# dropbox/rust-brotli

Measured on AMD Instinct MI355X. Metric: compress MB/s at q5 lgwin22, higher is better.
Workload: dtype u8; 1 GPU; 64 MiB synthetic English-like text per GPU, quality=5, lgwin=22, one-shot BrotliEncoderCompress (H6), input and stream resident in HBM; input_bytes_total=67108864, compressed_bytes=16370400

## Files before the change

### rust-brotli_amd/csrc/device_api.h

```cpp
#ifndef BROTLI_MI355X_DEVICE_API_H_
#define BROTLI_MI355X_DEVICE_API_H_

#include <stddef.h>
#include <stdint.h>

#include <vector>

#include "lz77_types.h"
#include "lz77_warmup.h"

#define BR_STREAM (::brotli_mi355x::dev_stream_flushed())

struct ihipStream_t;
namespace brotli_mi355x {

ihipStream_t* dev_stream_flushed();

void* dev_alloc(size_t bytes);
void* dev_alloc_uninit(size_t bytes);
#ifdef BROTLI_HOST_EMU
void dev_free(void* p);
#else
void dev_free(void* p) noexcept;
static_assert(noexcept(dev_free(nullptr)), "blocks are freed in destructors");
// ... 129 lines not shown
  uint16_t* stag;
  uint32_t* rows;
  void* checkpoints = nullptr;
  uint32_t* rows_changed_lo = nullptr;
  uint32_t* rows_changed_hi = nullptr;
  uint32_t splice_lists = 1;
  uint32_t* dict_items = nullptr;
  uint32_t* changed_slot;
  uint32_t* row_ctl;
  uint32_t* reset_counts;
  const uint32_t* count_base;
  uint32_t* run_end;
  unsigned long long* smask;
  uint32_t* gprev;
  uint8_t* big_tile;
  unsigned long long* pot = nullptr;
  uint32_t* pot_state = nullptr;
  uint32_t* pot_list = nullptr;
  uint32_t pot_list_cap = 0;
  uint32_t* flip_cells = nullptr;
  uint32_t cell_shift = 0, cells_per_key = 0;
  uint32_t changed_cap;
  uint16_t* sorted_tag[2] = {nullptr, nullptr};
  uint32_t* search_log = nullptr;
  uint32_t* recheck_list = nullptr;
  uint32_t* recheck_count = nullptr;
  uint32_t recheck_cap = 0;
  uint8_t* flags[2];
  Command* cmds;
  Segment* segments;
// ... 159 lines not shown
```

### rust-brotli_amd/csrc/lz77_kernels.hip

```cpp
#include <hip/hip_runtime.h>
#include <stdexcept>
#include <string>
#include <utility>
#include <string.h>
#include <mutex>
#include <vector>

#include "device_api.h"
#include "lz77_chain.h"
#include "lz77_rows.h"
#include "lz77_groups.h"
#include "device_scan.h"
#include "lz77_parse_args.h"
#include "zopfli_device.h"
#include "batch_greedy_device.h"

namespace brotli_mi355x {

void hip_check(hipError_t e, const char* what) {
  if (e == hipSuccess) return;
  (void)hipGetLastError();
  throw std::runtime_error(std::string("HIP error in ") + what + ": " + hipGetErrorString(e));
}

static constexpr uint32_t kSortTile = 4096;
// ... 654 lines not shown

__device__ __forceinline__ void row_changed(const RowArgs& a, uint32_t p) {
  if (p < a.geo.first_block_start) return;
  if (a.flags[p] & kFlagSearched) {
    mark_dirty(p, a.geo, a.dirty, a.rows_lo, a.rows_hi);
  } else {
    const uint32_t k = chain_in_front_if_near_boundary(p, a.geo);
    if (k != 0xffffffffu) {
      a.dirty[k] = 1;
      note_rows_changed(k, p, a.rows_lo, a.rows_hi);
    }
  }
}

static constexpr uint32_t kRowTile = kScanTile, kRowHalo = 256, kRowSpan = kRowTile + kRowHalo;
static constexpr uint32_t kMaxRowWalk = 2048;
static_assert(kRowSpan == 256 * 5, "five span entries per thread");

__global__ __launch_bounds__(256) void k_build_rows(RowArgs a) {
  if (a.conditional && a.ctl[kCtlNeedFull] == 0) return;
  if (a.conditional && a.validate && a.pot != nullptr && a.pot_state[0] != 0 && a.pot_state[2] == 0) return;
  typedef uint32_t u32x4 __attribute__((ext_vector_type(4)));
  __shared__ uint32_t s_pos[kRowSpan];
  __shared__ uint32_t s_tk[kRowSpan];
  __shared__ uint8_t s_fb[kRowSpan];
  __shared__ uint16_t s_rank[kRowSpan];
  __shared__ uint2 c_ent[kRowSpan];
  __shared__ uint32_t wave_sum[4];
  __shared__ alignas(16) uint32_t rowbuf[4][64 * kRowEntries];
  const uint32_t base = blockIdx.x * kRowTile;
// ... 223 lines not shown
        want = count != 0 && (count & 0xffffu) == 0;
      }
      if (want != ((f[j] & kSlotWrap) != 0)) {
        fbits[i] = (uint8_t)(f[j] ^ kSlotWrap);
        if (append) {
          const uint32_t real = *changed_count;
          const uint32_t at = real + atomicAdd(&ctl[kCtlVirtual], 1u);
          if (real <= cap && at < cap) changed_slot[at] = i; else atomicMax(&ctl[kCtlNeedFull], 1u);
        }
      }
    }
    g += f[j] & kSlotStored;
  }
}

__device__ __forceinline__ uint32_t slot_bits_of_flag(uint32_t flag) { return (flag & 1u) | ((flag & kFlagMasked) ? kSlotMasked : 0u); }

__global__ __launch_bounds__(256) void k_regather_fbits(const uint32_t* __restrict__ by_key, const uint8_t* __restrict__ flags, uint32_t n,
                                                         uint8_t* __restrict__ fbits, const uint32_t* __restrict__ ctl) {
  if (ctl[kCtlNeedFull] != 2) return;
  for (uint32_t i = blockIdx.x * blockDim.x + threadIdx.x; i < n; i += gridDim.x * blockDim.x)
    fbits[i] = (uint8_t)(slot_bits_of_flag(flags[by_key[i]]) | (fbits[i] & kSlotWrap));
}

__global__ __launch_bounds__(256) void k_apply_flips(const uint32_t* __restrict__ changed_pos, const uint32_t* __restrict__ changed_count,
                                                      uint32_t cap, const uint16_t* __restrict__ keys, const uint32_t* __restrict__ key_first,
                                                      const uint32_t* __restrict__ key_last, const uint32_t* __restrict__ by_key,
                                                      const uint8_t* __restrict__ flags_new, uint8_t* __restrict__ fbits,
                                                      uint32_t* __restrict__ changed_slot, uint32_t* __restrict__ ctl, uint32_t total_slots,
                                                      uint32_t all_keys) {
  const uint32_t i = blockIdx.x * blockDim.x + threadIdx.x;
  const uint32_t n = *changed_count;
  if (n > cap) {
    if (i == 0) {
      atomicMax(&ctl[kCtlNeedFull], 2u);
      atomicMax(&ctl[kCtlWrapKeyFlip], 1u);
    }
    return;
// ... 38 lines not shown
      const bool st = in && i != s && (a.fbits[i] & (kSlotStored | kSlotChanged)) == kSlotStored;
      const unsigned long long m = __ballot(st);
      const uint32_t before = (uint32_t)__popcll(m & ((1ull << threadIdx.x) - 1ull));
      bool build = in && stable + before < a.depth;
      if (use_pot && build) build = ((a.pot[i >> 6] >> (i & 63u)) & 1ull) != 0;
      if (build) {
        if (br_build_row(sl, a.rows, a.max_backward_limit, i, kf, a.depth, true, a.reset_pos, a.reset_vis)) row_changed(a, a.by_key[i]);
      }
      stable += (uint32_t)__popcll(m);
      const uint32_t cost = use_pot ? (__ballot(build) != 0 ? 64u : 4u) : 64u;
      if (threadIdx.x == 0) atomicAdd(&a.walk_counter[kCtlWalked], cost);
    }
  }
}

__global__ __launch_bounds__(256) void k_clear_flip_marks(const uint32_t* __restrict__ changed_slot, const uint32_t* __restrict__ changed_count,
                                                           uint32_t cap, uint8_t* __restrict__ fbits) {
  const uint32_t n = *changed_count;
  if (n > cap) return;
  for (uint32_t i = blockIdx.x * blockDim.x + threadIdx.x; i < n; i += gridDim.x * blockDim.x) fbits[changed_slot[i]] &= (uint8_t)~kSlotChanged;
}

static RowArgs row_args(const Lz77Params& P, const Lz77Buffers& B, int which, bool validate, const SegGeometry* geo, uint8_t* dirty_dev) {
  RowArgs a{};
  a.by_key = B.by_key;
  a.sorted_keys = B.sorted_keys;
  a.stag = B.stag;
  a.fbits = B.fbits;
  a.key_first = B.key_first;
  a.key_last = B.key_last;
  a.rows = B.rows;
  a.flags = B.flags[which];
  a.n = P.total_bytes;
  a.depth = 1u << P.block_bits;
  a.max_backward_limit = P.max_backward_limit;
// ... 14 lines not shown
  a.flip_cells = (validate && B.count_base == nullptr && P.reset_pos == 0) ? B.flip_cells : nullptr;
  a.cell_shift = B.cell_shift;
  a.cells_per_key = B.cells_per_key;
  a.cell_words = (uint32_t)(((size_t)65536 * B.cells_per_key) / 32);
  return a;
}

#if !defined(BR_POT_TABLE)
#define BR_POT_TABLE 8192
#define BR_POT_SHIFT 19
#endif
static constexpr uint32_t kPotTile = 1024, kPotHalo = 512, kPotSpan = kPotTile + kPotHalo, kPotTable = BR_POT_TABLE, kPotShift = BR_POT_SHIFT;
__global__ __launch_bounds__(256) void k_row_potential(const uint32_t* __restrict__ by_key, const uint16_t* __restrict__ sorted_keys,
                                                        const uint16_t* __restrict__ stag, uint32_t n, uint32_t max_backward_limit,
                                                        const uint32_t* __restrict__ ctl, uint32_t* __restrict__ pot_state,
                                                        unsigned long long* __restrict__ pot, uint32_t* __restrict__ pot_list, uint32_t list_cap) {
  if (ctl[kCtlNeedFull] == 0 || pot_state[0] != 0) return;
  __shared__ uint32_t s_val[kPotSpan];
  __shared__ uint32_t s_pos[kPotSpan];
  __shared__ uint32_t tab[kPotTable], tab2[kPotTable];
  __shared__ uint32_t s_count, s_base;
  const uint32_t lane = threadIdx.x & 63u;
  for (uint32_t h = threadIdx.x; h < kPotTable; h += 256) tab[h] = tab2[h] = 0;
  uint32_t gen = 0;
  for (uint32_t base = blockIdx.x * kPotTile; base < n; base += gridDim.x * kPotTile) {
    ++gen;
    const uint32_t lo = base >= kPotHalo ? base - kPotHalo : 0u;
    const uint32_t hi = min(base + kPotTile, n);
    const uint32_t span = hi - lo;
    __syncthreads();
    for (uint32_t e = threadIdx.x; e < span; e += 256) {
// ... 77 lines not shown
      }
      s_base = at;
    }
    __syncthreads();
    if (s_base != 0xffffffffu) {
      uint32_t at = s_base + (uint32_t)__shfl((int)wave_at, 0, 64);
#pragma unroll
      for (uint32_t r = 0; r < kPotTile / 256; ++r) {
        const unsigned long long m = masks[r];
        if ((m >> lane) & 1ull) pot_list[at + (uint32_t)__popcll(m & ((1ull << lane) - 1ull))] = base + r * 256 + threadIdx.x;
        at += (uint32_t)__popcll(m);
      }
    }
  }
}
__global__ __launch_bounds__(256) void k_validate_listed_rows(RowArgs a, const uint32_t* __restrict__ pot_list) {
  if (a.ctl[kCtlNeedFull] == 0 || a.pot_state[0] == 0 || a.pot_state[2] != 0) return;
  const uint32_t count = a.pot_state[1];
  SlotsInMemory sl{a.by_key, a.fbits, a.stag, a.smask, a.gprev};
  for (uint32_t t = blockIdx.x * blockDim.x + threadIdx.x; t < count; t += gridDim.x * blockDim.x) {
    const uint32_t i = pot_list[t];
    if (a.flip_cells != nullptr && a.flip_cells[a.cell_words] == 0) {
      const uint32_t p = a.by_key[i];
      const uint32_t first = (p > a.max_backward_limit ? p - a.max_backward_limit : 0u) >> a.cell_shift, last = p >> a.cell_shift;
      const uint32_t key = a.sorted_keys[i];
      const uint32_t cell0 = key * a.cells_per_key;
      bool any = a.key_last[key] - a.key_first[key] >= 65536u;
      for (uint32_t c = cell0 + first; c <= cell0 + last; ++c) any = any || ((a.flip_cells[c >> 5] >> (c & 31u)) & 1u) != 0;
      if (!any) continue;
    }
    const uint32_t kf = a.key_first[a.sorted_keys[i]];
    if (br_build_row(sl, a.rows, a.max_backward_limit, i, kf, a.depth, true, a.reset_pos, a.reset_vis)) row_changed(a, a.by_key[i]);
  }
}
__global__ void k_row_potential_ready(const uint32_t* __restrict__ ctl, uint32_t* __restrict__ pot_state) {
  if (ctl[kCtlNeedFull] != 0 && threadIdx.x == 0 && blockIdx.x == 0) pot_state[0] = 1;
}

__global__ __launch_bounds__(256) void k_slot_masks(const uint8_t* __restrict__ fbits, uint32_t n, unsigned long long* __restrict__ smask,
                                                     uint32_t* __restrict__ glast) {
  const uint32_t groups = (n + 63) / 64;
  for (uint32_t g = blockIdx.x * blockDim.x + threadIdx.x; g < groups; g += gridDim.x * blockDim.x) {
    unsigned long long m = 0;
    const uint4* src = (const uint4*)(fbits + (size_t)g * 64);
#pragma unroll
    for (uint32_t q = 0; q < 4; ++q) {
      const uint4 v = src[q];
      const uint32_t w[4] = {v.x, v.y, v.z, v.w};
#pragma unroll
      for (uint32_t k = 0; k < 4; ++k) {
        const uint32_t b = w[k] & 0x01010101u;
        const uint32_t nib = (b | (b >> 7) | (b >> 14) | (b >> 21)) & 0xfu;
        m |= (unsigned long long)nib << (q * 16 + k * 4);
      }
    }
    if ((size_t)g * 64 + 64 > n) m &= (1ull << (n - g * 64)) - 1ull;
    smask[g] = m;
    glast[g] = m ? g * 64 + 64 - (uint32_t)__builtin_clzll(m) : 0u;
  }
}

__global__ __launch_bounds__(256) void k_maxscan_tiles(uint32_t* __restrict__ data, uint32_t n, uint32_t* __restrict__ tile_max) {
  __shared__ uint32_t wave_max[4];
  const uint32_t base = blockIdx.x * kScanTile + threadIdx.x * 4;
  uint32_t v[4];
#pragma unroll
  for (int j = 0; j < 4; ++j) v[j] = (base + j < n) ? data[base + j] : 0;
  const uint32_t local = max(max(v[0], v[1]), max(v[2], v[3]));
  uint32_t x = local;
  const int lane = threadIdx.x & 63, w = threadIdx.x >> 6;
#pragma unroll
  for (int off = 1; off < 64; off <<= 1) {
    const uint32_t y = __shfl_up(x, off, 64);
// ... 17 lines not shown
  const uint32_t add = tile_before[blockIdx.x];
#pragma unroll
  for (int j = 0; j < 4; ++j)
    if (base + j < n) data[base + j] = max(data[base + j], add);
}
static void exclusive_maxscan_u32(uint32_t* data, uint32_t n, uint32_t* scratch) {
  if (n == 0) return;
  const uint32_t tiles = (n + kScanTile - 1) / kScanTile;
  hipLaunchKernelGGL(k_maxscan_tiles, dim3(tiles), dim3(256), 0, BR_STREAM, data, n, tiles > 1 ? scratch : (uint32_t*)nullptr);
  if (tiles > 1) {
    exclusive_maxscan_u32(scratch, tiles, scratch + tiles);
    hipLaunchKernelGGL(k_maxscan_add, dim3(tiles), dim3(256), 0, BR_STREAM, data, n, scratch);
  }
}

static void launch_slot_masks(const Lz77Params& P, const Lz77Buffers& B) {
  const uint32_t n = P.total_bytes;
  const uint32_t groups = (n + 63) / 64;
  uint32_t blocks = (groups + 255) / 256;
  if (blocks > 4096) blocks = 4096;
  hipLaunchKernelGGL(k_slot_masks, dim3(blocks), dim3(256), 0, BR_STREAM, B.fbits, n, B.smask, B.gprev);
  uint32_t* scratch = (uint32_t*)B.sort_tmp + ((size_t)n / kScanTile + 4096);
  exclusive_maxscan_u32(B.gprev, groups, scratch);
}

static void launch_wrap_marks(const Lz77Params& P, const Lz77Buffers& B, bool append) {
  const uint32_t n = P.total_bytes;
  const uint32_t tiles = (n + kRowTile - 1) / kRowTile;
  uint32_t* tile_sums = (uint32_t*)B.sort_tmp;
  uint32_t* scratch = tile_sums + tiles + 64;
  const uint32_t* skip_unless = append ? B.row_ctl + kCtlWrapKeyFlip : (const uint32_t*)nullptr;
  hipLaunchKernelGGL(k_fbits_tile_sums, dim3(tiles), dim3(256), 0, BR_STREAM, B.fbits, n, B.big_tile, tile_sums, skip_unless);
  exclusive_scan_u32(tile_sums, tiles, scratch);
  const bool all_keys = B.count_base != nullptr || P.reset_pos != 0;
  hipLaunchKernelGGL(k_row_key_bases, dim3(256), dim3(256), 0, BR_STREAM, B.fbits, tile_sums, B.key_first, B.key_last, B.key_base,
                     all_keys ? 1u : 0u, skip_unless);
  hipLaunchKernelGGL(k_mark_wraps, dim3(tiles), dim3(256), 0, BR_STREAM, B.fbits, n, B.big_tile, tile_sums, B.sorted_keys, B.key_first, B.key_last,
                     B.key_base, append ? 1u : 0u, B.changed_slot, B.changed_count, B.changed_cap, B.row_ctl, B.count_base, B.by_key, P.reset_pos,
                     B.reset_counts);
}

void lz77_rows_init(const Lz77Params& P, const Lz77Buffers& B, int which, const RankInitialHint* initial, bool has_big_keys) {
  const uint32_t n = P.total_bytes;
  if (n == 0) return;
  if ((1u << P.block_bits) > kRowEntries) throw std::runtime_error("candidate rows: ring deeper than a row");
// ... 6 lines not shown
    ig.total_bytes = n;
    ig.prefix_stored_end = (initial->prefix_is_dictionary && P.prefix_bytes > P.htl - 1) ? P.prefix_bytes - (P.htl - 1) : 0;
  }
  const uint32_t tiles = (n + kScanTile - 1) / kScanTile;
  uint32_t* tile_sums = (uint32_t*)B.sort_tmp;
  hipLaunchKernelGGL(k_rank_gather, dim3(tiles), dim3(256), 0, BR_STREAM, B.by_key, B.flags[which], n, B.fbits, tile_sums, ig,
                     P.masked_from != kNeverMasked ? 1u : 0u);
  dev_memset(B.row_ctl, 0, kCtlWords * 4);
  if (P.reset_pos) lz77_key_counts(P, B, which, P.reset_vis, B.reset_counts, false);
  if (has_big_keys) {
    dev_memset(B.big_tile, 0, tiles + 64);
    hipLaunchKernelGGL(k_flag_big_tiles, dim3(256), dim3(256), 0, BR_STREAM, B.key_first, B.key_last, B.big_tile,
                       (B.count_base || P.reset_pos) ? 1u : 0u);
    launch_wrap_marks(P, B, false);
  }
  launch_slot_masks(P, B);
  RowArgs a = row_args(P, B, which, false, nullptr, nullptr);
  hipLaunchKernelGGL(k_build_rows, dim3((n + kRowTile - 1) / kRowTile), dim3(256), 0, BR_STREAM, a);
  HIP_CHECK(hipGetLastError());
}

void lz77_rows_update(const Lz77Params& P, const Lz77Buffers& B, int prev, int next, const SegGeometry& geo, uint8_t* dirty_dev,
                      bool has_big_keys) {
  const uint32_t n = P.total_bytes;
  if (n == 0) return;
  const uint32_t cap = B.changed_cap;
  dev_memset(B.row_ctl, 0, kCtlWords * 4);
  const uint32_t flip_blocks = (cap + 255) / 256;
  hipLaunchKernelGGL(k_apply_flips, dim3(flip_blocks), dim3(256), 0, BR_STREAM, B.changed_keys, B.changed_count, cap, B.keys, B.key_first,
                     B.key_last, B.by_key, B.flags[next], B.fbits, B.changed_slot, B.row_ctl, n,
                     (B.count_base != nullptr || P.reset_pos != 0) ? 1u : 0u);
  uint32_t gather_blocks = (n + 255) / 256;
  if (gather_blocks > 8192) gather_blocks = 8192;
  hipLaunchKernelGGL(k_regather_fbits, dim3(gather_blocks), dim3(256), 0, BR_STREAM, B.by_key, B.flags[next], n, B.fbits, B.row_ctl);
  if (P.reset_pos) lz77_key_counts(P, B, next, P.reset_vis, B.reset_counts, false);
  if (has_big_keys) launch_wrap_marks(P, B, true);
  launch_slot_masks(P, B);
  RowArgs a = row_args(P, B, next, true, &geo, dirty_dev);
  hipLaunchKernelGGL(k_update_rows, dim3(cap < 65536u ? cap : 65536u), dim3(64), 0, BR_STREAM, a, B.changed_slot, B.changed_count, B.keys);
  a.conditional = 1;
  if (B.pot) {
    uint32_t pot_blocks = (n + kPotTile - 1) / kPotTile;
    if (pot_blocks > 8192u) pot_blocks = 8192u;
    hipLaunchKernelGGL(k_row_potential, dim3(pot_blocks), dim3(256), 0, BR_STREAM, B.by_key, B.sorted_keys, B.stag, n, P.max_backward_limit,
                       B.row_ctl, B.pot_state, B.pot, B.pot_list, B.pot_list_cap);
    hipLaunchKernelGGL(k_row_potential_ready, dim3(1), dim3(64), 0, BR_STREAM, B.row_ctl, B.pot_state);
    hipLaunchKernelGGL(k_validate_listed_rows, dim3(2048), dim3(256), 0, BR_STREAM, a, B.pot_list);
  }
  hipLaunchKernelGGL(k_build_rows, dim3((n + kRowTile - 1) / kRowTile), dim3(256), 0, BR_STREAM, a);
  hipLaunchKernelGGL(k_clear_flip_marks, dim3(flip_blocks < 1024u ? flip_blocks : 1024u), dim3(256), 0, BR_STREAM, B.changed_slot, B.changed_count,
                     cap, B.fbits);
  HIP_CHECK(hipGetLastError());
  (void)prev;
}

__global__ __launch_bounds__(64) void k_key_counts(const uint32_t* __restrict__ by_key, const uint8_t* __restrict__ flags,
                                                    const uint32_t* __restrict__ key_first, const uint32_t* __restrict__ key_last,
                                                    const uint32_t* __restrict__ base, uint32_t upto, uint32_t* __restrict__ out) {
  const uint32_t key = blockIdx.x;
  uint32_t local = 0;
  for (uint32_t i = key_first[key] + threadIdx.x; i < key_last[key]; i += 64) {
    const uint32_t p = by_key[i];
    if (p < upto) local += flags[p] & 1u;
  }
  for (int off = 32; off > 0; off >>= 1) local += __shfl_down(local, off, 64);
  if (threadIdx.x == 0) out[key] = local + (base ? base[key] : 0u);
// ... 1612 lines not shown
```

### rust-brotli_amd/csrc/lz77_stage.cpp

```cpp
#include "lz77_stage.h"
#include "timeline.h"

#include <math.h>
#include <stdio.h>
#include <stdlib.h>
#include <string.h>

#include <algorithm>
#include <chrono>
#include <map>
#include <stdexcept>
#include <string>

#include "host_entropy.h"

#include <cmath>

#if defined(BROTLI_HOST_EMU)
#include "lz77_warmup_emu.inc"
#endif

namespace brotli_mi355x {

void Lz77Stage::Release() {
// ... 204 lines not shown
      L_.rank[i] = mem_.uninit<uint32_t>((M + 1) * 4 + 64);
      L_.entry[i] = mem_.uninit<uint32_t>(M * 4 + 64);
    }
    if (live_verify_) {
      B_.search_log = mem_.zeroed<uint32_t>(M * kSearchLogWords * 4 + 64);
      B_.recheck_cap = (uint32_t)(M + 4096);
      B_.recheck_list = mem_.uninit<uint32_t>((size_t)B_.recheck_cap * 4 + 64);
      B_.recheck_count = mem_.zeroed<uint32_t>(64);
    }
    L_.changed_key = mem_.zeroed<uint8_t>(65536 + 64);
    B_.changed_cap = kChangedCap;
    B_.changed_keys = mem_.zeroed<uint32_t>((size_t)kChangedCap * 4);
  } else
  if (use_rows_) {
    B_.changed_cap = (uint32_t)std::max<size_t>(kChangedCap, M / 32);
    B_.changed_keys = mem_.uninit<uint32_t>((size_t)B_.changed_cap * 4 + 64);
    B_.changed_slot = mem_.uninit<uint32_t>((size_t)B_.changed_cap * 4 + 64);
    B_.row_ctl = mem_.zeroed<uint32_t>(64);
    B_.big_tile = mem_.zeroed<uint8_t>(M / 1024 + 128);
    B_.smask = mem_.uninit<unsigned long long>((M / 64 + 2) * 8 + 64);
    B_.gprev = mem_.uninit<uint32_t>((M / 64 + 2) * 4 + 64);
    if (getenv("BROTLI_MI355X_NO_POTENTIAL_MASK") == nullptr) {
      B_.pot = mem_.uninit<unsigned long long>((M / 64 + 2) * 8 + 64);
      B_.pot_state = mem_.zeroed<uint32_t>(64);
      B_.pot_list_cap = (uint32_t)(M / 16 + 1024);
      B_.pot_list = mem_.uninit<uint32_t>((size_t)B_.pot_list_cap * 4 + 64);
      if (getenv("BROTLI_MI355X_NO_FLIP_CELLS") == nullptr) {
        uint32_t shift = 8;
        while (shift < 31 && (1u << shift) < P_.max_backward_limit + 1u) ++shift;
        while (shift < 31 && (M >> shift) + 2 > 1024) ++shift;
        B_.cell_shift = shift;
        B_.cells_per_key = (uint32_t)(M >> shift) + 2;
        B_.flip_cells = mem_.zeroed<uint32_t>((size_t)65536 * B_.cells_per_key / 8 + 64);
      }
// ... 947 lines not shown
    }
  } else {
    mem_.drop(B_.run_end);
  }
  has_big_keys_ = false;
  for (uint32_t key = 0; key < 65536 && !has_big_keys_; ++key) has_big_keys_ = key_last_[key] - key_first_[key] >= 65536u;
  if (carry_ && carry_->valid && carry_->key_counts.size() == 65536) {
    if (!count_base_dev_) count_base_dev_ = mem_.zeroed<uint32_t>(65536 * 4);
    dev_h2d(count_base_dev_, carry_->key_counts.data(), 65536 * 4);
    B_.count_base = count_base_dev_;
    has_big_keys_ = true;
  } else {
    B_.count_base = nullptr;
  }
  if (P_.reset_pos) has_big_keys_ = true;
  tm.stop(&stats_.ms_sort);
  timeline().stamp("rounds");
  RunRounds(true);
  tm.stop(&stats_.ms_resolve);
  timeline().stamp("gather");
  Gather();
  timeline().stamp("gathered");
  tm.stop(&stats_.ms_gather);
  total.stop(&stats_.ms_total);
  if (prof)
    fprintf(stderr, "lz77 stage: keys %.2f sort %.2f init %.2f warmup %.2f rank %.2f parse %.2f resolve %.2f gather %.2f | total %.2f ms, rounds %u\n",
            stats_.ms_keys, stats_.ms_sort, stats_.ms_init, stats_.ms_warmup, stats_.ms_rank, stats_.ms_parse, stats_.ms_resolve, stats_.ms_gather,
            stats_.ms_total, (unsigned)stats_.rounds);
  if (prof) fprintf(stderr, "  host: Resolve() %.2f ms, recheck + scheduling %.2f ms\n", host_resolve_ms_, host_schedule_ms_);
  host_resolve_ms_ = host_schedule_ms_ = 0;
// ... 589 lines not shown
  const uint32_t nseg = (uint32_t)segments_.size();
  resolve_incremental_ = true;
  block_records_valid_ = false;
  touch_all_ = true;
  block_touched_.assign(block_segment_bytes_.size(), 0);
  InitFlags();
  tm.stop(&stats_.ms_init);
  const bool selftest = getenv("BROTLI_MI355X_SELFTEST") != nullptr;
  const bool selftest_rows_every_update = getenv("BROTLI_MI355X_SELFTEST_ROWS") != nullptr;
  if (selftest) SelfTestSort();
  int which = 0, rbuf = 0;
  {
    RankInitialHint hint{segments_[0].blk_start, block_bytes_, (carry_ && carry_->valid) ? 0u : 1u};
    if (use_rows_) {
      lz77_rows_init(P_, B_, which, &hint, has_big_keys_);
    } else {
      lz77_rank_flags(P_, B_, which, rbuf, &hint);
    }
  }
  InitEntries();
  tm.stop(&stats_.ms_rank);
  timeline().stamp("index-queued");
  if (selftest) {
    if (use_rows_) SelfTestRows(which); else SelfTestRank(which, rbuf);
  }
  SegGeometry geo{};
  geo.prefix_bytes = P_.prefix_bytes;
  geo.first_block_start = segments_[0].blk_start;
  geo.block_bytes = block_bytes_;
  geo.num_blocks = (uint32_t)block_segment_bytes_.size();
// ... 578 lines not shown
    }
    if (i + 1 == n || skeys[i + 1] != skeys[i]) {
      if (key_last_[skeys[i]] != i + 1) throw std::runtime_error("selftest: key_last mismatch for key " + std::to_string(skeys[i]));
    }
    const bool plain_counters = B_.count_base == nullptr && P_.reset_pos == 0;
    const uint32_t visible = std::min(local & 0xffffu, local);
    if (info[2 * (size_t)p] != first + local || (plain_counters && info[2 * (size_t)p + 1] != visible))
      throw std::runtime_error("selftest: info mismatch at slot " + std::to_string(i));
    if (flags[p] & 1) {
      if (sorted[first + local] != p) throw std::runtime_error("selftest: sorted mismatch at slot " + std::to_string(i));
      local++;
    }
  }
}

void Lz77Stage::SelfTestRows(int which) {
  const uint32_t n = P_.total_bytes;
  std::vector<uint16_t> skeys(n);
  std::vector<uint32_t> by_key(n), rows((size_t)n * kRowEntries);
  std::vector<uint8_t> flags(n), fbits(n), text((size_t)n + 64, 0);
  dev_sync();
  dev_d2h(skeys.data(), B_.sorted_keys, (size_t)n * 2);
  dev_d2h(by_key.data(), B_.by_key, (size_t)n * 4);
  dev_d2h(rows.data(), B_.rows, (size_t)n * kRowEntries * 4);
  dev_d2h(flags.data(), B_.flags[which], n);
  dev_d2h(fbits.data(), B_.fbits, n);
  dev_d2h(text.data(), B_.text, n);
  auto tag = [&](uint32_t p) {
    uint32_t v;
    memcpy(&v, text.data() + p, 4);
    return (uint32_t)((v * 0x9E3779B1u) >> 16);
  };
  const uint32_t depth = 1u << P_.block_bits;
  uint32_t first = 0, stored_before = 0, local_before = 0, since_reset = 0;
  for (uint32_t i = 0; i < n; ++i) {
    const uint32_t p = by_key[i];
    if (i == 0 || skeys[i - 1] != skeys[i]) {
      first = i;
      stored_before = B_.count_base ? carry_->key_counts[skeys[i]] : 0u;
      local_before = 0;
      since_reset = 0;
    }
    const uint32_t counter = (P_.reset_pos != 0 && p >= P_.reset_pos) ? since_reset : stored_before;
    if ((fbits[i] & 1) != (flags[p] & 1)) throw std::runtime_error("selftest: fbits mismatch at slot " + std::to_string(i));
    if (fbits[i] & 2) throw std::runtime_error("selftest: leftover change mark at slot " + std::to_string(i));
    {
      const bool big = P_.reset_pos != 0 || B_.count_base != nullptr || key_last_[skeys[i]] - key_first_[skeys[i]] >= 65536u;
      const bool want_wrap = big && counter != 0 && (counter & 0xffffu) == 0;
      if (want_wrap != ((fbits[i] & 4) != 0)) throw std::runtime_error("selftest: wrap mark mismatch at slot " + std::to_string(i));
    }
    const uint32_t max_backward = std::min(p, P_.max_backward_limit);
    const uint32_t d = std::min(depth, counter & 0xffffu);
    const uint32_t oldest = p >= P_.reset_pos ? P_.reset_vis : 0u;
    std::vector<uint32_t> want;
    uint32_t seen = 0;
    for (uint32_t j = i; j > first && seen < d;) {
      --j;
      if (!(flags[by_key[j]] & 1)) continue;
      if (p - by_key[j] > max_backward || by_key[j] < oldest) break;
      ++seen;
      if (tag(by_key[j]) == tag(p)) want.push_back(by_key[j]);
    }
    for (size_t c = 0; c <= want.size() && c < kRowEntries; ++c) {
      const uint32_t have = rows[(size_t)p * kRowEntries + c];
      const uint32_t expect = c < want.size() ? want[c] : kRowEnd;
      if (have != expect)
        throw std::runtime_error("selftest: row of position " + std::to_string(p) + " entry " + std::to_string(c) + ": " + std::to_string(have) +
                                 " instead of " + std::to_string(expect));
    }
    stored_before += flags[p] & 1;
    local_before += flags[p] & 1;
    if (P_.reset_pos != 0 && p >= P_.reset_vis) since_reset += flags[p] & 1;
  }
// ... 102 lines not shown
```

### rust-brotli_amd/csrc/lz77_stage.h

```cpp
#ifndef BROTLI_MI355X_LZ77_STAGE_H_
#define BROTLI_MI355X_LZ77_STAGE_H_

#include <stdint.h>
#include <map>
#include <memory>
#include <utility>
#include <vector>

#include "device_api.h"
#include "encoder_params.h"
#include "quick_api.h"

namespace brotli_mi355x {

struct MetaBlockPlan {
  uint32_t start;
  uint32_t end;
  uint32_t cmd_offset;
  uint32_t n_cmds;
  uint32_t n_literals;
  bool uncompressed;
  bool is_last;
  int32_t dist_cache_after[4];
  int32_t saved_dist_cache[4];
// ... 109 lines not shown
    PinnedArray<SegExit> wexits;
    DevBlocks mem;
    uint32_t count = 0;
    bool dict_dead = false, whole_input = true;
    bool launched = true;
    int mark = 0;
  };
  uint32_t WarmupPlan(WarmupJob* job, uint32_t first_seg, uint32_t end_seg, bool dict_dead, const std::vector<uint8_t>* only_after_dirty);
  void Warmup(uint32_t first_seg, bool dict_dead, int which, int rbuf, const std::vector<uint8_t>* only_after_dirty);
  void WarmupBegin(WarmupJob* job, uint32_t first_seg, uint32_t end_seg, bool dict_dead, int which, int rbuf,
                   const std::vector<uint8_t>* only_after_dirty, int mark);
  void WarmupEnd(WarmupJob* job);
  void SelfTestSort();
  void SelfTestRank(int which, int rbuf);
  void SelfTestRows(int which);
  bool FetchShouldCompress();
  bool ResolvePass(bool final_pass, bool incremental);
  void SetupCommon(bool with_sort_tmp);
  void Release();

  EncoderParams params_;
  Lz77Params P_{};
  DevBlocks mem_;
  Lz77Buffers B_{};
  LiveBuffers L_{};
  bool use_live_ = false;
  bool use_zopfli_ = false;
  ZopfliJob Z_{};
  uint32_t* zsnap_buckets_ = nullptr;
  uint32_t* zsnap_forest_ = nullptr;
// ... 106 lines not shown
  std::vector<Patch> patches_prev_;
  std::vector<TrailingInsert> trailing_prev_;
  std::vector<Carry> carries_prev_;
  std::vector<uint8_t> block_touched_;
  bool block_records_valid_ = false, touch_all_ = true, resolve_incremental_ = false;
  uint32_t resolve_blocks_skipped_ = 0;
  void TouchSegment(uint32_t k) {
    if (!block_touched_.empty()) block_touched_[segments_[k].block_index] = 1;
  }
  std::vector<uint8_t> dirty_entry_;
  uint32_t dict_death_seg_ = 0xffffffffu;
  uint32_t dict_flips_ = 0;
  uint32_t* count_base_dev_ = nullptr;
  bool use_rows_ = false;
  bool has_big_keys_ = false;
};

}
#endif
```

Baseline: 4862 MB/s.

## Restrict wrap marking to big-key tiles and fuse slot-mask regather and skip scan

Builds a host-side list of row tiles covered by keys with at least 65536 slots. The incremental wrap-mark pass now sums, scans and marks only those tiles instead of every tile. Folds the fbits regather into k_slot_masks, replaces the generic max-scan with a per-tile max plus a dedicated skip-pointer kernel, and folds the flip-mark clear and potential-ready flag into existing kernels to cut launches. It also shrinks the k_update_rows grid and adds selftest checks, at the cost of more complex indexing logic and a host-to-device copy of the run list.

Result: no change. 4849 MB/s (-0.3%).

```diff
diff --git a/rust-brotli_amd/csrc/device_api.h b/rust-brotli_amd/csrc/device_api.h
--- a/rust-brotli_amd/csrc/device_api.h
+++ b/rust-brotli_amd/csrc/device_api.h
@@ -167,6 +167,8 @@
   unsigned long long* smask;
   uint32_t* gprev;
   uint8_t* big_tile;
+  uint32_t* wrap_runs;
+  uint32_t wrap_run_count, wrap_listed;
   unsigned long long* pot = nullptr;
   uint32_t* pot_state = nullptr;
   uint32_t* pot_list = nullptr;
diff --git a/rust-brotli_amd/csrc/lz77_kernels.hip b/rust-brotli_amd/csrc/lz77_kernels.hip
--- a/rust-brotli_amd/csrc/lz77_kernels.hip
+++ b/rust-brotli_amd/csrc/lz77_kernels.hip
@@ -9,6 +9,7 @@
 #include "device_api.h"
 #include "lz77_chain.h"
 #include "lz77_rows.h"
+#include "lz77_wrap.h"
 #include "lz77_groups.h"
 #include "device_scan.h"
 #include "lz77_parse_args.h"
@@ -693,6 +694,7 @@
 }
 
 static constexpr uint32_t kRowTile = kScanTile, kRowHalo = 256, kRowSpan = kRowTile + kRowHalo;
+static constexpr uint32_t kIdleGrid = 8192;
 static constexpr uint32_t kMaxRowWalk = 2048;
 static_assert(kRowSpan == 256 * 5, "five span entries per thread");
 
@@ -946,14 +948,81 @@
   }
 }
 
+static_assert(kWrapTile == kRowTile, "lz77_wrap.h counts in row tiles");
+
+__global__ __launch_bounds__(256) void k_wrap_tile_sums(const uint8_t* __restrict__ fbits, uint32_t n, const uint16_t* __restrict__ sorted_keys,
+                                                         const uint32_t* __restrict__ key_first, const uint32_t* __restrict__ key_last,
+                                                         WrapRuns w, uint32_t* __restrict__ sums, const uint32_t* __restrict__ ctl) {
+  if (ctl[kCtlWrapKeyFlip] == 0) return;
+  __shared__ uint32_t wave_sum[4];
+  for (uint32_t j = blockIdx.x; j < w.listed; j += gridDim.x) {
+    const WrapTileKeys k = br_wrap_tile_keys(br_wrap_listed_tile(w, j), n, sorted_keys, key_first, key_last);
+    const uint32_t base = k.lo + threadIdx.x * 4;
+    uint32_t local = 0;
+    if (base < k.hi) {
+      const uint32_t v = *(const uint32_t*)(fbits + base);
+#pragma unroll
+      for (uint32_t q = 0; q < 4; ++q)
+        if (base + q < k.hi) local += br_wrap_sum_term(k, base + q, (v >> (8 * q)) & 0xffu);
+    }
+    const uint32_t total = block_sum_256(local, wave_sum);
+    if (threadIdx.x == 0) sums[j] = total;
+  }
+}
+
+__global__ __launch_bounds__(256) void k_mark_wraps_listed(uint8_t* __restrict__ fbits, uint32_t n, const uint16_t* __restrict__ sorted_keys,
+                                                            const uint32_t* __restrict__ key_first, const uint32_t* __restrict__ key_last,
+                                                            WrapRuns w, const uint32_t* __restrict__ local, const uint32_t* __restrict__ block_sum,
+                                                            uint32_t* __restrict__ changed_slot,
+                                                            const uint32_t* __restrict__ changed_count, uint32_t cap, uint32_t* __restrict__ ctl) {
+  if (ctl[kCtlWrapKeyFlip] == 0) return;
+  __shared__ uint32_t wave_sum[4];
+  __shared__ uint32_t between_sum[4];
+  const int lane = threadIdx.x & 63, wv = threadIdx.x >> 6;
+  for (uint32_t j = blockIdx.x; j < w.listed; j += gridDim.x) {
+    const WrapTileKeys k = br_wrap_tile_keys(br_wrap_listed_tile(w, j), n, sorted_keys, key_first, key_last);
+    uint32_t head_base = 0;
+    if (k.head) {
+      uint32_t part = 0;
+      for (uint32_t b = br_wrap_head_first(k, j) / kWrapScanBlock + threadIdx.x; b < j / kWrapScanBlock; b += 256) part += block_sum[b];
+      head_base = br_wrap_head_base(k, local, block_sum_256(part, between_sum), j);
+    }
+    const uint32_t base = k.lo + threadIdx.x * 4;
+    uint32_t f[4], mine = 0;
+#pragma unroll
+    for (int q = 0; q < 4; ++q) {
+      f[q] = base + q < k.hi ? fbits[base + q] : 0u;
+      mine += f[q] & kSlotStored;
+    }
+    uint32_t x = mine;
+#pragma unroll
+    for (int off = 1; off < 64; off <<= 1) {
+      const uint32_t y = __shfl_up(x, off, 64);
+      if (lane >= off) x += y;
+    }
+    if (lane == 63) wave_sum[wv] = x;
+    __syncthreads();
+    uint32_t g = x - mine;
+    for (int i = 0; i < wv; ++i) g += wave_sum[i];
+#pragma unroll
+    for (int q = 0; q < 4; ++q) {
+      const uint32_t i = base + q;
+      if (i < k.hi) {
+        const bool want = br_wrap_wanted(k, i, g, head_base);
+        if (want != ((f[q] & kSlotWrap) != 0)) {
+          fbits[i] = (uint8_t)(f[q] ^ kSlotWrap);
+          const uint32_t real = *changed_count;
+          const uint32_t at = real + atomicAdd(&ctl[kCtlVirtual], 1u);
+          if (real <= cap && at < cap) changed_slot[at] = i; else atomicMax(&ctl[kCtlNeedFull], 1u);
+        }
+      }
+      g += f[q] & kSlotStored;
+    }
+    __syncthreads();
+  }
+}
+
 __device__ __forceinline__ uint32_t slot_bits_of_flag(uint32_t flag) { return (flag & 1u) | ((flag & kFlagMasked) ? kSlotMasked : 0u); }
-
-__global__ __launch_bounds__(256) void k_regather_fbits(const uint32_t* __restrict__ by_key, const uint8_t* __restrict__ flags, uint32_t n,
-                                                         uint8_t* __restrict__ fbits, const uint32_t* __restrict__ ctl) {
-  if (ctl[kCtlNeedFull] != 2) return;
-  for (uint32_t i = blockIdx.x * blockDim.x + threadIdx.x; i < n; i += gridDim.x * blockDim.x)
-    fbits[i] = (uint8_t)(slot_bits_of_flag(flags[by_key[i]]) | (fbits[i] & kSlotWrap));
-}
 
 __global__ __launch_bounds__(256) void k_apply_flips(const uint32_t* __restrict__ changed_pos, const uint32_t* __restrict__ changed_count,
                                                       uint32_t cap, const uint16_t* __restrict__ keys, const uint32_t* __restrict__ key_first,
@@ -1022,11 +1091,15 @@
   }
 }
 
-__global__ __launch_bounds__(256) void k_clear_flip_marks(const uint32_t* __restrict__ changed_slot, const uint32_t* __restrict__ changed_count,
-                                                           uint32_t cap, uint8_t* __restrict__ fbits) {
+__device__ __forceinline__ void clear_flip_marks(const uint32_t* __restrict__ changed_slot, const uint32_t* __restrict__ changed_count,
+                                                 uint32_t cap, uint8_t* __restrict__ fbits) {
   const uint32_t n = *changed_count;
   if (n > cap) return;
   for (uint32_t i = blockIdx.x * blockDim.x + threadIdx.x; i < n; i += gridDim.x * blockDim.x) fbits[changed_slot[i]] &= (uint8_t)~kSlotChanged;
+}
+__global__ __launch_bounds__(256) void k_clear_flip_marks(const uint32_t* __restrict__ changed_slot, const uint32_t* __restrict__ changed_count,
+                                                           uint32_t cap, uint8_t* __restrict__ fbits) {
+  clear_flip_marks(changed_slot, changed_count, cap, fbits);
 }
 
 static RowArgs row_args(const Lz77Params& P, const Lz77Buffers& B, int which, bool validate, const SegGeometry* geo, uint8_t* dirty_dev) {
@@ -1071,7 +1144,10 @@
 __global__ __launch_bounds__(256) void k_row_potential(const uint32_t* __restrict__ by_key, const uint16_t* __restrict__ sorted_keys,
                                                         const uint16_t* __restrict__ stag, uint32_t n, uint32_t max_backward_limit,
                                                         const uint32_t* __restrict__ ctl, uint32_t* __restrict__ pot_state,
-                                                        unsigned long long* __restrict__ pot, uint32_t* __restrict__ pot_list, uint32_t list_cap) {
+                                                        unsigned long long* __restrict__ pot, uint32_t* __restrict__ pot_list, uint32_t list_cap,
+                                                        const uint32_t* __restrict__ changed_slot, const uint32_t* __restrict__ changed_count,
+                                                        uint32_t changed_cap, uint8_t* __restrict__ fbits) {
+  clear_flip_marks(changed_slot, changed_count, changed_cap, fbits);
   if (ctl[kCtlNeedFull] == 0 || pot_state[0] != 0) return;
   __shared__ uint32_t s_val[kPotSpan];
   __shared__ uint32_t s_pos[kPotSpan];
@@ -1179,8 +1255,10 @@
     }
   }
 }
-__global__ __launch_bounds__(256) void k_validate_listed_rows(RowArgs a, const uint32_t* __restrict__ pot_list) {
-  if (a.ctl[kCtlNeedFull] == 0 || a.pot_state[0] == 0 || a.pot_state[2] != 0) return;
+__global__ __launch_bounds__(256) void k_validate_listed_rows(RowArgs a, const uint32_t* __restrict__ pot_list, uint32_t* pot_state_out) {
+  if (a.ctl[kCtlNeedFull] == 0) return;
+  if (blockIdx.x == 0 && threadIdx.x == 0) pot_state_out[0] = 1;
+  if (a.pot_state[2] != 0) return;
   const uint32_t count = a.pot_state[1];
   SlotsInMemory sl{a.by_key, a.fbits, a.stag, a.smask, a.gprev};
   for (uint32_t t = blockIdx.x * blockDim.x + threadIdx.x; t < count; t += gridDim.x * blockDim.x) {
@@ -1198,14 +1276,32 @@
     if (br_build_row(sl, a.rows, a.max_backward_limit, i, kf, a.depth, true, a.reset_pos, a.reset_vis)) row_changed(a, a.by_key[i]);
   }
 }
-__global__ void k_row_potential_ready(const uint32_t* __restrict__ ctl, uint32_t* __restrict__ pot_state) {
-  if (ctl[kCtlNeedFull] != 0 && threadIdx.x == 0 && blockIdx.x == 0) pot_state[0] = 1;
-}
-
-__global__ __launch_bounds__(256) void k_slot_masks(const uint8_t* __restrict__ fbits, uint32_t n, unsigned long long* __restrict__ smask,
-                                                     uint32_t* __restrict__ glast) {
+
+static constexpr uint32_t kMaskTile = 256;
+
+__device__ __forceinline__ uint32_t block_max_256(uint32_t v, uint32_t* wave_max) {
+  for (int off = 32; off > 0; off >>= 1) v = max(v, (uint32_t)__shfl_down(v, off, 64));
+  __syncthreads();
+  if ((threadIdx.x & 63) == 0) wave_max[threadIdx.x >> 6] = v;
+  __syncthreads();
+  return max(max(wave_max[0], wave_max[1]), max(wave_max[2], wave_max[3]));
+}
+
+__global__ __launch_bounds__(256) void k_slot_masks(uint8_t* __restrict__ fbits, uint32_t n, unsigned long long* __restrict__ smask,
+                                                     uint32_t* __restrict__ glast, uint32_t* __restrict__ tile_last,
+                                                     const uint32_t* __restrict__ ctl, const uint32_t* __restrict__ by_key,
+                                                     const uint8_t* __restrict__ flags) {
+  __shared__ uint32_t wave_max[4];
   const uint32_t groups = (n + 63) / 64;
-  for (uint32_t g = blockIdx.x * blockDim.x + threadIdx.x; g < groups; g += gridDim.x * blockDim.x) {
+  if (ctl != nullptr && ctl[kCtlNeedFull] == 2) {
+    const uint32_t lo = blockIdx.x * kMaskTile * 64;
+    const uint32_t hi = n - lo < kMaskTile * 64 ? n : lo + kMaskTile * 64;
+    for (uint32_t i = lo + threadIdx.x; i < hi; i += 256) fbits[i] = (uint8_t)(slot_bits_of_flag(flags[by_key[i]]) | (fbits[i] & kSlotWrap));
+    __syncthreads();
+  }
+  const uint32_t g = blockIdx.x * kMaskTile + threadIdx.x;
+  uint32_t last = 0;
+  if (g < groups) {
     unsigned long long m = 0;
     const uint4* src = (const uint4*)(fbits + (size_t)g * 64);
 #pragma unroll
@@ -1221,7 +1317,46 @@
     }
     if ((size_t)g * 64 + 64 > n) m &= (1ull << (n - g * 64)) - 1ull;
     smask[g] = m;
-    glast[g] = m ? g * 64 + 64 - (uint32_t)__builtin_clzll(m) : 0u;
+    last = m ? g * 64 + 64 - (uint32_t)__builtin_clzll(m) : 0u;
+    glast[g] = last;
+  }
+  const uint32_t top = block_max_256(last, wave_max);
+  if (threadIdx.x == 0) tile_last[blockIdx.x] = top;
+}
+
+__global__ __launch_bounds__(256) void k_skip_pointers(uint32_t* __restrict__ gprev, uint32_t groups, const uint32_t* __restrict__ tile_last,
+                                                        uint32_t tiles, uint32_t tiles_per_block) {
+  __shared__ uint32_t wave_max[4];
+  const uint32_t first = blockIdx.x * tiles_per_block;
+  const uint32_t end = tiles - first < tiles_per_block ? tiles : first + tiles_per_block;
+  uint32_t carry = 0;
+  for (uint32_t top = first; top > 0 && carry == 0; top = top > 4096u ? top - 4096u : 0u) {
+    uint32_t v = 0;
+    for (uint32_t q = 0; q < 16; ++q) {
+      const uint32_t back = q * 256 + threadIdx.x;
+      if (top > back) v = max(v, tile_last[top - 1 - back]);
+    }
+    carry = block_max_256(v, wave_max);
+  }
+  const int lane = threadIdx.x & 63, w = threadIdx.x >> 6;
+  for (uint32_t tile = first; tile < end; ++tile) {
+    __syncthreads();
+    const uint32_t g = tile * kMaskTile + threadIdx.x;
+    const uint32_t v = g < groups ? gprev[g] : 0u;
+    uint32_t x = v;
+#pragma unroll
+    for (int off = 1; off < 64; off <<= 1) {
+      const uint32_t y = __shfl_up(x, off, 64);
+      if (lane >= off) x = max(x, y);
+    }
+    if (lane == 63) wave_max[w] = x;
+    __syncthreads();
+    uint32_t before = carry;
+    for (int i = 0; i < w; ++i) before = max(before, wave_max[i]);
+    const uint32_t prev_lane = __shfl_up(x, 1, 64);
+    if (lane > 0) before = max(before, prev_lane);
+    if (g < groups) gprev[g] = before;
+    carry = max(max(carry, max(wave_max[0], wave_max[1])), max(wave_max[2], wave_max[3]));
   }
 }
 
@@ -1269,14 +1404,16 @@
   }
 }
 
-static void launch_slot_masks(const Lz77Params& P, const Lz77Buffers& B) {
+static void launch_slot_masks(const Lz77Params& P, const Lz77Buffers& B, const uint8_t* regather_from) {
   const uint32_t n = P.total_bytes;
   const uint32_t groups = (n + 63) / 64;
-  uint32_t blocks = (groups + 255) / 256;
-  if (blocks > 4096) blocks = 4096;
-  hipLaunchKernelGGL(k_slot_masks, dim3(blocks), dim3(256), 0, BR_STREAM, B.fbits, n, B.smask, B.gprev);
-  uint32_t* scratch = (uint32_t*)B.sort_tmp + ((size_t)n / kScanTile + 4096);
-  exclusive_maxscan_u32(B.gprev, groups, scratch);
+  const uint32_t blocks = (groups + kMaskTile - 1) / kMaskTile;
+  uint32_t* tile_last = (uint32_t*)B.sort_tmp + ((size_t)n / kScanTile + 4096);
+  hipLaunchKernelGGL(k_slot_masks, dim3(blocks), dim3(256), 0, BR_STREAM, B.fbits, n, B.smask, B.gprev, tile_last,
+                     regather_from ? B.row_ctl : (const uint32_t*)nullptr, B.by_key, regather_from);
+  const uint32_t tiles_per_block = (blocks + 4095) / 4096;
+  hipLaunchKernelGGL(k_skip_pointers, dim3((blocks + tiles_per_block - 1) / tiles_per_block), dim3(256), 0, BR_STREAM, B.gprev, groups, tile_last,
+                     blocks, tiles_per_block);
 }
 
 static void launch_wrap_marks(const Lz77Params& P, const Lz77Buffers& B, bool append) {
@@ -1284,6 +1421,17 @@
   const uint32_t tiles = (n + kRowTile - 1) / kRowTile;
   uint32_t* tile_sums = (uint32_t*)B.sort_tmp;
   uint32_t* scratch = tile_sums + tiles + 64;
+  if (append && B.wrap_listed != 0) {
+    const WrapRuns w{B.wrap_runs, B.wrap_run_count, B.wrap_listed};
+    const uint32_t grid = w.listed < 65536u ? w.listed : 65536u;
+    hipLaunchKernelGGL(k_wrap_tile_sums, dim3(grid), dim3(256), 0, BR_STREAM, B.fbits, n, B.sorted_keys, B.key_first, B.key_last, w, tile_sums,
+                       B.row_ctl);
+    static_assert(kWrapScanBlock == kScanTile, "br_wrap_head_base counts in scan tiles");
+    hipLaunchKernelGGL(k_scan_tiles, dim3((w.listed + kScanTile - 1) / kScanTile), dim3(256), 0, BR_STREAM, tile_sums, w.listed, scratch);
+    hipLaunchKernelGGL(k_mark_wraps_listed, dim3(grid), dim3(256), 0, BR_STREAM, B.fbits, n, B.sorted_keys, B.key_first, B.key_last, w, tile_sums,
+                       scratch, B.changed_slot, B.changed_count, B.changed_cap, B.row_ctl);
+    return;
+  }
   const uint32_t* skip_unless = append ? B.row_ctl + kCtlWrapKeyFlip : (const uint32_t*)nullptr;
   hipLaunchKernelGGL(k_fbits_tile_sums, dim3(tiles), dim3(256), 0, BR_STREAM, B.fbits, n, B.big_tile, tile_sums, skip_unless);
   exclusive_scan_u32(tile_sums, tiles, scratch);
@@ -1320,7 +1468,7 @@
                        (B.count_base || P.reset_pos) ? 1u : 0u);
     launch_wrap_marks(P, B, false);
   }
-  launch_slot_masks(P, B);
+  launch_slot_masks(P, B, nullptr);
   RowArgs a = row_args(P, B, which, false, nullptr, nullptr);
   hipLaunchKernelGGL(k_build_rows, dim3((n + kRowTile - 1) / kRowTile), dim3(256), 0, BR_STREAM, a);
   HIP_CHECK(hipGetLastError());
@@ -1336,26 +1484,23 @@
   hipLaunchKernelGGL(k_apply_flips, dim3(flip_blocks), dim3(256), 0, BR_STREAM, B.changed_keys, B.changed_count, cap, B.keys, B.key_first,
                      B.key_last, B.by_key, B.flags[next], B.fbits, B.changed_slot, B.row_ctl, n,
                      (B.count_base != nullptr || P.reset_pos != 0) ? 1u : 0u);
-  uint32_t gather_blocks = (n + 255) / 256;
-  if (gather_blocks > 8192) gather_blocks = 8192;
-  hipLaunchKernelGGL(k_regather_fbits, dim3(gather_blocks), dim3(256), 0, BR_STREAM, B.by_key, B.flags[next], n, B.fbits, B.row_ctl);
+  launch_slot_masks(P, B, B.flags[next]);
   if (P.reset_pos) lz77_key_counts(P, B, next, P.reset_vis, B.reset_counts, false);
   if (has_big_keys) launch_wrap_marks(P, B, true);
-  launch_slot_masks(P, B);
   RowArgs a = row_args(P, B, next, true, &geo, dirty_dev);
-  hipLaunchKernelGGL(k_update_rows, dim3(cap < 65536u ? cap : 65536u), dim3(64), 0, BR_STREAM, a, B.changed_slot, B.changed_count, B.keys);
+  hipLaunchKernelGGL(k_update_rows, dim3(cap < kIdleGrid ? cap : kIdleGrid), dim3(64), 0, BR_STREAM, a, B.changed_slot, B.changed_count, B.keys);
   a.conditional = 1;
   if (B.pot) {
     uint32_t pot_blocks = (n + kPotTile - 1) / kPotTile;
     if (pot_blocks > 8192u) pot_blocks = 8192u;
     hipLaunchKernelGGL(k_row_potential, dim3(pot_blocks), dim3(256), 0, BR_STREAM, B.by_key, B.sorted_keys, B.stag, n, P.max_backward_limit,
-                       B.row_ctl, B.pot_state, B.pot, B.pot_list, B.pot_list_cap);
-    hipLaunchKernelGGL(k_row_potential_ready, dim3(1), dim3(64), 0, BR_STREAM, B.row_ctl, B.pot_state);
-    hipLaunchKernelGGL(k_validate_listed_rows, dim3(2048), dim3(256), 0, BR_STREAM, a, B.pot_list);
+                       B.row_ctl, B.pot_state, B.pot, B.pot_list, B.pot_list_cap, B.changed_slot, B.changed_count, cap, B.fbits);
+    hipLaunchKernelGGL(k_validate_listed_rows, dim3(2048), dim3(256), 0, BR_STREAM, a, B.pot_list, B.pot_state);
   }
   hipLaunchKernelGGL(k_build_rows, dim3((n + kRowTile - 1) / kRowTile), dim3(256), 0, BR_STREAM, a);
-  hipLaunchKernelGGL(k_clear_flip_marks, dim3(flip_blocks < 1024u ? flip_blocks : 1024u), dim3(256), 0, BR_STREAM, B.changed_slot, B.changed_count,
-                     cap, B.fbits);
+  if (!B.pot)
+    hipLaunchKernelGGL(k_clear_flip_marks, dim3(flip_blocks < 1024u ? flip_blocks : 1024u), dim3(256), 0, BR_STREAM, B.changed_slot, B.changed_count,
+                       cap, B.fbits);
   HIP_CHECK(hipGetLastError());
   (void)prev;
 }
diff --git a/rust-brotli_amd/csrc/lz77_stage.cpp b/rust-brotli_amd/csrc/lz77_stage.cpp
--- a/rust-brotli_amd/csrc/lz77_stage.cpp
+++ b/rust-brotli_amd/csrc/lz77_stage.cpp
@@ -1,4 +1,5 @@
 #include "lz77_stage.h"
+#include "lz77_wrap_list.h"
 #include "timeline.h"
 
 #include <math.h>
@@ -242,10 +243,12 @@
   } else
   if (use_rows_) {
     B_.changed_cap = (uint32_t)std::max<size_t>(kChangedCap, M / 32);
+    if (const char* cap = getenv("BROTLI_MI355X_TEST_CHANGED_CAP")) B_.changed_cap = (uint32_t)std::max(1, atoi(cap));
     B_.changed_keys = mem_.uninit<uint32_t>((size_t)B_.changed_cap * 4 + 64);
     B_.changed_slot = mem_.uninit<uint32_t>((size_t)B_.changed_cap * 4 + 64);
     B_.row_ctl = mem_.zeroed<uint32_t>(64);
     B_.big_tile = mem_.zeroed<uint8_t>(M / 1024 + 128);
+    B_.wrap_runs = mem_.uninit<uint32_t>((M / 65536 + 2) * 8 + 64);
     B_.smask = mem_.uninit<unsigned long long>((M / 64 + 2) * 8 + 64);
     B_.gprev = mem_.uninit<uint32_t>((M / 64 + 2) * 4 + 64);
     if (getenv("BROTLI_MI355X_NO_POTENTIAL_MASK") == nullptr) {
@@ -1223,6 +1226,7 @@
     B_.count_base = nullptr;
   }
   if (P_.reset_pos) has_big_keys_ = true;
+  B_.wrap_run_count = B_.wrap_listed = 0;
   tm.stop(&stats_.ms_sort);
   timeline().stamp("rounds");
   RunRounds(true);
@@ -1842,6 +1846,7 @@
     RankInitialHint hint{segments_[0].blk_start, block_bytes_, (carry_ && carry_->valid) ? 0u : 1u};
     if (use_rows_) {
       lz77_rows_init(P_, B_, which, &hint, has_big_keys_);
+      ListWrapTiles();
     } else {
       lz77_rank_flags(P_, B_, which, rbuf, &hint);
     }
@@ -2450,6 +2455,19 @@
   }
 }
 
+void Lz77Stage::ListWrapTiles() {
+  if (B_.wrap_listed != 0) return;
+  if (!has_big_keys_ || B_.count_base != nullptr || P_.reset_pos != 0) return;
+  wrap_runs_.clear();
+  uint32_t listed = 0, next_tile = 0;
+  for (uint32_t key = 0; key < 65536; ++key)
+    if (key_last_[key] - key_first_[key] >= kWrapKeySlots) br_wrap_list_key(&wrap_runs_, &listed, &next_tile, key_first_[key], key_last_[key]);
+  if (listed == 0) return;
+  dev_h2d(B_.wrap_runs, wrap_runs_.data(), wrap_runs_.size() * 4);
+  B_.wrap_run_count = (uint32_t)(wrap_runs_.size() / 2);
+  B_.wrap_listed = listed;
+}
+
 void Lz77Stage::SelfTestRows(int which) {
   const uint32_t n = P_.total_bytes;
   std::vector<uint16_t> skeys(n);
@@ -2467,7 +2485,29 @@
     memcpy(&v, text.data() + p, 4);
     return (uint32_t)((v * 0x9E3779B1u) >> 16);
   };
+  if (B_.smask != nullptr && B_.gprev != nullptr) {
+    const uint32_t groups = (n + 63) / 64;
+    std::vector<unsigned long long> smask(groups);
+    std::vector<uint32_t> gprev(groups);
+    dev_d2h(smask.data(), B_.smask, (size_t)groups * 8);
+    dev_d2h(gprev.data(), B_.gprev, (size_t)groups * 4);
+    uint32_t last = 0;
+    for (uint32_t g = 0; g < groups; ++g) {
+      unsigned long long m = 0;
+      const uint32_t end = std::min(n, g * 64 + 64);
+      for (uint32_t i = g * 64; i < end; ++i) m |= (unsigned long long)(fbits[i] & 1) << (i & 63u);
+      if (smask[g] != m) throw std::runtime_error("selftest: stored-bit mask mismatch at group " + std::to_string(g));
+      if (gprev[g] != last) throw std::runtime_error("selftest: skip pointer mismatch at group " + std::to_string(g));
+      for (uint32_t i = g * 64; i < end; ++i)
+        if (fbits[i] & 1) last = i + 1;
+    }
+  }
   const uint32_t depth = 1u << P_.block_bits;
+  std::vector<uint32_t> prev_stored(n);
+  for (uint32_t i = 0, last = 0; i < n; ++i) {
+    prev_stored[i] = last;
+    if (flags[by_key[i]] & 1) last = i + 1;
+  }
   uint32_t first = 0, stored_before = 0, local_before = 0, since_reset = 0;
   for (uint32_t i = 0; i < n; ++i) {
     const uint32_t p = by_key[i];
@@ -2490,9 +2530,9 @@
     const uint32_t oldest = p >= P_.reset_pos ? P_.reset_vis : 0u;
     std::vector<uint32_t> want;
     uint32_t seen = 0;
-    for (uint32_t j = i; j > first && seen < d;) {
-      --j;
-      if (!(flags[by_key[j]] & 1)) continue;
+    for (uint32_t j = i; seen < d;) {
+      if (prev_stored[j] <= first) break;
+      j = prev_stored[j] - 1;
       if (p - by_key[j] > max_backward || by_key[j] < oldest) break;
       ++seen;
       if (tag(by_key[j]) == tag(p)) want.push_back(by_key[j]);
diff --git a/rust-brotli_amd/csrc/lz77_stage.h b/rust-brotli_amd/csrc/lz77_stage.h
--- a/rust-brotli_amd/csrc/lz77_stage.h
+++ b/rust-brotli_amd/csrc/lz77_stage.h
@@ -147,6 +147,7 @@
   void SelfTestSort();
   void SelfTestRank(int which, int rbuf);
   void SelfTestRows(int which);
+  void ListWrapTiles();
   bool FetchShouldCompress();
   bool ResolvePass(bool final_pass, bool incremental);
   void SetupCommon(bool with_sort_tmp);
@@ -283,6 +284,7 @@
   uint32_t* count_base_dev_ = nullptr;
   bool use_rows_ = false;
   bool has_big_keys_ = false;
+  std::vector<uint32_t> wrap_runs_;
 };
 
 }
diff --git a/rust-brotli_amd/csrc/lz77_wrap.h b/rust-brotli_amd/csrc/lz77_wrap.h
--- /dev/null
+++ b/rust-brotli_amd/csrc/lz77_wrap.h
@@ -0,0 +1,58 @@
+#ifndef BROTLI_MI355X_LZ77_WRAP_H_
+#define BROTLI_MI355X_LZ77_WRAP_H_
+
+#include "lz77_rows.h"
+#include "lz77_wrap_list.h"
+
+namespace brotli_mi355x {
+
+BR_DEV uint32_t br_wrap_listed_tile(const WrapRuns& w, uint32_t j) {
+  uint32_t lo = 0, hi = w.count;
+  while (lo + 1 < hi) {
+    const uint32_t mid = lo + (hi - lo) / 2;
+    if (w.runs[2 * mid + 1] <= j) lo = mid; else hi = mid;
+  }
+  return w.runs[2 * lo] + (j - w.runs[2 * lo + 1]);
+}
+
+struct WrapTileKeys {
+  uint32_t lo, hi;
+  uint32_t head_key, tail_key;
+  uint32_t head_end;
+  uint32_t tail_first;
+  uint32_t head_tiles;
+  bool head;
+};
+
+BR_DEV WrapTileKeys br_wrap_tile_keys(uint32_t tile, uint32_t n, const uint16_t* sorted_keys, const uint32_t* key_first, const uint32_t* key_last) {
+  WrapTileKeys k;
+  k.lo = tile * kWrapTile;
+  k.hi = k.lo + kWrapTile < n ? k.lo + kWrapTile : n;
+  k.head_key = sorted_keys[k.lo];
+  k.tail_key = sorted_keys[k.hi - 1];
+  const uint32_t hf = key_first[k.head_key], hl = key_last[k.head_key];
+  k.head = hl - hf >= kWrapKeySlots;
+  k.head_end = hl < k.hi ? hl : k.hi;
+  k.head_tiles = tile - hf / kWrapTile;
+  k.tail_first = k.tail_key == k.head_key ? k.lo : key_first[k.tail_key];
+  return k;
+}
+
+BR_DEV uint32_t br_wrap_sum_term(const WrapTileKeys& k, uint32_t i, uint32_t fb) { return i >= k.tail_first ? (fb & kSlotStored) : 0u; }
+
+static constexpr uint32_t kWrapScanBlock = 1024;
+BR_DEV uint32_t br_wrap_head_first(const WrapTileKeys& k, uint32_t j) {
+  return j - (k.head_tiles < j ? k.head_tiles : j);
+}
+BR_DEV uint32_t br_wrap_head_base(const WrapTileKeys& k, const uint32_t* local, uint32_t between, uint32_t j) {
+  return local[j] - local[br_wrap_head_first(k, j)] + between;
+}
+
+BR_DEV bool br_wrap_wanted(const WrapTileKeys& k, uint32_t i, uint32_t before, uint32_t head_base) {
+  if (!k.head || i >= k.head_end) return false;
+  const uint32_t count = head_base + before;
+  return count != 0 && (count & 0xffffu) == 0;
+}
+
+}
+#endif
diff --git a/rust-brotli_amd/csrc/lz77_wrap_list.h b/rust-brotli_amd/csrc/lz77_wrap_list.h
--- /dev/null
+++ b/rust-brotli_amd/csrc/lz77_wrap_list.h
@@ -0,0 +1,30 @@
+#ifndef BROTLI_MI355X_LZ77_WRAP_LIST_H_
+#define BROTLI_MI355X_LZ77_WRAP_LIST_H_
+
+#include <stdint.h>
+
+namespace brotli_mi355x {
+
+static constexpr uint32_t kWrapTile = 1024;
+static constexpr uint32_t kWrapKeySlots = 65536;
+
+struct WrapRuns {
+  const uint32_t* runs;
+  uint32_t count, listed;
+};
+
+template <typename Vec>
+inline void br_wrap_list_key(Vec* runs, uint32_t* listed, uint32_t* next_tile, uint32_t first, uint32_t last) {
+  const uint32_t t0 = first / kWrapTile, t1 = (last - 1) / kWrapTile;
+  uint32_t start = *next_tile;
+  if (runs->empty() || t0 > *next_tile) {
+    runs->push_back(t0);
+    runs->push_back(*listed);
+    start = t0;
+  }
+  *listed += t1 + 1 - start;
+  *next_tile = t1 + 1;
+}
+
+}
+#endif
```
